# pscoro/JPEG-XL-Lossy-Image-Compression-Thesis

Measured on AMD Instinct MI355X. Metric: MPix/s VarDCT encode @ d1.0, 8K RGB, higher is better.
Workload: dtype f32; 1 GPU; 8k 7680x4320 RGB8 (synth_rgb8), VarDCT d1 e7, cjxl defaults (JXG_FLAGS_CJXL_DEFAULTS: Gaborish + EPF + masking AQ), proposals=0, ans-coded, 1 frame(s) per step, 2 distinct frames cycled, streaming entry points (jxg_submit_rgb8_device / jxg_receive, one host thread); global_batch=1, parallelism=frame-dp1

## Files before the change

jpeg-xl-lossy-image-compression-thesis_amd/csrc/jxg_encode.cpp:

```cpp
#include "jxg_ctx.h"

#include <cstdlib>
#include <cstring>

#include "jxg_codes.h"
#include "jxg_tables.h"

namespace jxg {

static void build_rows(const Frame& f, const Plan& P, std::vector<LfRow>& rows,
                       std::vector<LfChunk>& chunks, std::vector<uint32_t>& schunks) {
  rows.clear();
  chunks.clear();
  schunks.clear();
  auto add = [&](uint32_t lg, uint16_t stream, uint16_t ch, uint32_t y, uint32_t width) {
    for (uint32_t x0 = 0; x0 < width; x0 += kLfSeg) {
      const uint32_t wseg = std::min(kLfSeg, width - x0);
      const uint32_t sid = lg * 2 + stream;
      if (chunks.empty() || chunks.back().sid != sid || chunks.back().nrows == kLfChunkRows ||
          chunks.back().nsamp + wseg > kLfChunkSamples)
        chunks.push_back({(uint32_t)rows.size(), 0, sid, 0});
      chunks.back().nrows++;
      chunks.back().nsamp += wseg;
      rows.push_back({lg, stream, ch, y, x0, wseg, sid});
    }
  };
  for (uint32_t lg = 0; lg < f.nlf; lg++) {
    const uint32_t bx0 = (lg % f.lfxs) * 256, by0 = (lg / f.lfxs) * 256;
    const uint32_t bw = std::min(256u, f.bxs - bx0), bh = std::min(256u, f.bys - by0);
    const bool own = P.owns_lf(lg);
    schunks.push_back((uint32_t)chunks.size());
    if (own)
      for (uint16_t ch = 0; ch < 3; ch++)
        for (uint32_t y = 0; y < bh; y++) add(lg, 0, ch, y, bw);
    schunks.push_back((uint32_t)chunks.size());
    if (own) {
      const uint32_t cw = (bw + 7) / 8, chh = (bh + 7) / 8;
      for (uint16_t ch = 0; ch < 2; ch++)
        for (uint32_t y = 0; y < chh; y++) add(lg, 1, ch, y, cw);
      for (uint32_t y = 0; y < 2; y++) add(lg, 1, 2, y, bw * bh);
      for (uint32_t y = 0; y < bh; y++) add(lg, 1, 3, y, bw);
    }
  }
  schunks.push_back((uint32_t)chunks.size());
}

jxg_status wait_emission(Ctx* c, Job& J) {
  (void)J;
  JXG_HIP(hipStreamSynchronize(c->stream));
  return JXG_OK;
}

jxg_status stage_alloc(Ctx* c, Job& J) {
  hipStream_t s = c->stream;
  const jxg_params& P = c->params;
  const Frame& f = J.f;
  const size_t nb = (size_t)f.bxs * f.bys;
  J.homog = (P.proposals & 3u) != 0;
  J.ans = (P.flags & JXG_FLAG_ANS) != 0;
  J.lf = lf_code(P.flags, P.distance);
  jxg_status st = init_constants(c);
  if (st) return st;
  JXG_HIP(c->acs.ensure(nb));
  JXG_HIP(c->qf.ensure(nb));
  JXG_HIP(c->nz.ensure(nb * 3));
  JXG_HIP(c->dc.ensure(nb * 3));
  JXG_HIP(c->ac.ensure(nb * 192));
  if (J.homog) JXG_HIP(c->homog.ensure(nb * 3));
  J.max_s = P.effort >= 6 ? 8 : (P.effort >= 5 ? 4 : 0);
  const uint32_t ntiles = f.tiles_x * f.tiles_y;
  JXG_HIP(c->cmap.ensure((size_t)ntiles * 2));
  if (J.max_s) {
    JXG_HIP(c->ent.ensure(nb));
    JXG_HIP(c->xyb_tiles.ensure((size_t)ntiles * 3 * 4096));
    JXG_HIP(c->mcost.ensure((size_t)ntiles * kNumShapes * 32));
    JXG_HIP(c->mwork.ensure(1 + (size_t)ntiles * kNumShapes));
  }
  const bool new_plan = c->rows_w != J.w || c->rows_h != J.h || c->rows_rank != J.plan.rank ||
                        c->rows_world != J.plan.world;
  if (!J.plan.tiles.empty()) {
    JXG_HIP(c->tile_list.ensure(J.plan.tiles.size()));
    if (new_plan)
      JXG_HIP(hipMemcpyAsync(c->tile_list.p, J.plan.tiles.data(), J.plan.tiles.size() * 4,
                             hipMemcpyHostToDevice, s));
  }
  if (!J.plan.lf_mine.empty()) {
    JXG_HIP(c->lf_mine.ensure(J.plan.lf_mine.size()));
    if (new_plan)
      JXG_HIP(hipMemcpyAsync(c->lf_mine.p, J.plan.lf_mine.data(), J.plan.lf_mine.size(),
                             hipMemcpyHostToDevice, s));
  }
  JXG_HIP(c->vb.ensure((size_t)f.nlf * 65536));
  J.nstreams = f.nlf * 2;
  {
    const EncArenas::Layouts L = c->declare(f, J.plan.ng());
    JXG_HIP(c->stat.ensure(c->stat_bytes));
    JXG_HIP(c->h_stat.ensure(c->stat_bytes));
    JXG_HIP(c->up.ensure(c->up_bytes));
    JXG_HIP(c->h_up.ensure(c->up_bytes));
    JXG_HIP(c->bits.ensure(c->bits_bytes));
    JXG_HIP(c->h_bits.ensure(c->bits_bytes));
    L.stat.commit(c->stat.p, c->h_stat.p);
    L.up.commit(c->up.p, c->h_up.p);
    L.bits.commit(c->bits.p, c->h_bits.p);
  }
  if (new_plan) {
    build_rows(f, J.plan, c->rows_h_cache, c->chunks_h_cache, c->schunks_cache);
    c->rows_w = J.w;
    c->rows_h = J.h;
    c->rows_rank = J.plan.rank;
    c->rows_world = J.plan.world;
  }
  J.nrows = (uint32_t)c->rows_h_cache.size();
  J.nchunks = (uint32_t)c->chunks_h_cache.size();
  const uint32_t nstreams = J.nstreams;
  JXG_HIP(c->rows.ensure(J.nrows));
  JXG_HIP(c->lfchunks.ensure(J.nchunks));
  JXG_HIP(c->lfstatus.ensure(J.nchunks));
  JXG_HIP(c->stream_chunks.ensure(nstreams + 1));
  if (new_plan) {
    if (J.nrows)
      JXG_HIP(hipMemcpyAsync(c->rows.p, c->rows_h_cache.data(), J.nrows * sizeof(LfRow),
                             hipMemcpyHostToDevice, s));
    if (J.nchunks)
      JXG_HIP(hipMemcpyAsync(c->lfchunks.p, c->chunks_h_cache.data(), J.nchunks * sizeof(LfChunk),
                             hipMemcpyHostToDevice, s));
    JXG_HIP(hipMemcpyAsync(c->stream_chunks.p, c->schunks_cache.data(),
                           c->schunks_cache.size() * 4, hipMemcpyHostToDevice, s));
  }
// ... 748 lines not shown
```

jpeg-xl-lossy-image-compression-thesis_amd/csrc/jxg_kernels.h:

```cpp
#pragma once
#include <cmath>
#include <hip/hip_runtime.h>
#include <stddef.h>
#include <stdint.h>

#include "jxg_acmodel.h"
#include "jxg_decode_core.h"

namespace jxg {

constexpr uint32_t kMaxBatch = 4;
template <class A>
struct Batch {
  A a[kMaxBatch];
};
template <class A>
inline Batch<A> make_batch(const A* a, uint32_t k) {
  Batch<A> b{};
  for (uint32_t i = 0; i < k && i < kMaxBatch; i++) b.a[i] = a[i];
  return b;
}

struct FrontArgs {
  const uint8_t* rgb;
  uint32_t w, h;
  size_t stride;
  uint32_t bxs, bys, xp, yp, tiles_x;
  float distance;
  int effort;
  uint32_t proposals;
  int h1_int;
  int gab;
  float qf_base, inv_g;
  uint32_t G;
  float dc_mul[3], dc_step[3];
  uint8_t* acs;
  uint8_t* qf;
  int32_t* dc;
  int16_t* ac;
  uint16_t* nz;
  float* homog;
  float* ent;
  float* xyb_out;
  const uint32_t* tile_list;
  int8_t* cmap;
  uint32_t ntiles_all;
  uint4* zero;
  uint32_t zero_quads;
  const uint8_t* qf_in;
};
struct AqArgs {
  const uint8_t* rgb;
  uint32_t w, h;
  size_t stride;
  uint32_t xp, yp, bxs, bys, tiles_x;
  const float* lut;
  float ew[4];
  float mul, add, inv_g;
  uint8_t* qf;
  const uint32_t* tile_list;
};
void launch_aq(const AqArgs* a, uint32_t k, uint32_t ntiles, hipStream_t s);

constexpr int kNumKinds = 6;
constexpr int kKindOff[kNumKinds + 1] = {0, 128, 384, 896, 1920, 3968, 8064};
constexpr int kNumShapes = 9;
constexpr int kShapeOff[kNumShapes + 1] = {0, 128, 256, 512, 1024, 1536, 2560, 4608, 6656, 10752};
struct MergeArgs {
  const float* xyb;
  uint32_t bxs, bys, tiles_x, ntiles;
  const uint32_t* tile_list;
  uint32_t proposals;
  int max_s;
  uint32_t G;
  float dc_mul[3], dc_step[3];
  float* ent;
  const float* homog;
  uint8_t* acs;
  uint8_t* qf;
  int32_t* dc;
  int16_t* ac;
  uint16_t* nz;
  float* cost;
  const float* wk;
  const float* iwy;
  const float* sdk;
  const uint16_t* nat;
  uint32_t* work;
  uint32_t nwrite;
  const int8_t* cmap;
  uint32_t ntiles_all;
};
constexpr int kBigKindOff[5] = {0, 8192, 24576, 57344, 122880};
constexpr uint32_t kBigSlots = 512;
constexpr size_t kBigPlanes = 3 * 65536;
constexpr size_t kBigTabW = 0, kBigTabSd = 3 * 122880, kBigTabIw = 6 * 122880,
                 kBigTabLeeC = 7 * 122880, kBigTabLeeS = kBigTabLeeC + 9 * 128,
                 kBigTabLlfP = kBigTabLeeS + 9 * 256, kBigTabLlfIb = kBigTabLlfP + 6 * 32,
                 kBigTabFloats = kBigTabLlfIb + 6 * 32 * 32;
struct BigArgs {
  MergeArgs m;
  const float* tab;
  const uint16_t* nat;
  float* scratch;
  uint32_t slots;
  float* cost;
  uint32_t* work;
  uint32_t* kinds;
  const uint32_t* glist;
  uint32_t g0, ng, gxs;
};
hipError_t launch_big(const BigArgs* a, uint32_t k, hipStream_t s);

struct VbArgs {
  const uint8_t* acs;
  uint32_t bxs, bys, lfxs;
  const uint8_t* lf_mine;
  uint32_t* vb;
  uint32_t* count;
};
// ... 213 lines not shown
```

jpeg-xl-lossy-image-compression-thesis_amd/csrc/jxg_merge.hip:

```cpp
#include <float.h>

#include <cstdio>
#include <type_traits>

#include "jxg_device.h"
#include "jxg_kernels.h"
#include "jxg_lee_tables.h"

namespace jxg {

__constant__ float c_llf_p[4 * 8];
__constant__ float c_llf_ib[4 * 64];

constexpr int kMThreads = 256;
#ifndef JXG_MERGE_WPE
#define JXG_MERGE_WPE 4
#endif
#ifndef JXG_MERGE_WRITE_WPE
#define JXG_MERGE_WRITE_WPE 3
#endif
constexpr int kMS = 65;
constexpr int kMPlane = 64 * kMS;

template <int N>
// ... 47 lines not shown
    for (int k = 0; k < H - 1; k++) out(k, (t[k] + t[k + 1]) * kLeeS[l][2 * k + 1]);
    out(H - 1, t[H - 1] * kLeeS[l][N - 1]);
  }
}
template <class T>
__device__ __forceinline__ T dct64_first(T xi, T xm, int i, int h) {
  return dctN_first<64>(xi, xm, i, h);
}
template <class T, class Out>
__device__ __forceinline__ void dct64_rest(T* t, int h, Out out) {
  dctN_rest<64>(t, h, out);
}

#ifdef JXG_MERGE_PROFILE
__device__ unsigned long long g_mprof[16][8];
#define MPROF_MARK(k)                                                 \
  do {                                                                \
    if (!WRITE && threadIdx.x == 0) {                                 \
      const unsigned long long now_ = __builtin_readcyclecounter();   \
      if ((k) > 0) atomicAdd(&g_mprof[P.si][(k)], now_ - mprof_t0);   \
      mprof_t0 = now_;                                                \
    }                                                                 \
  } while (0)
#else
#define MPROF_MARK(k) \
  do {                \
  } while (0)
#endif

struct ShapeDesc {
  int type, lcy, lcx;
  float tmul;
};
constexpr ShapeDesc kShapes[kNumShapes] = {
    {6, 1, 0, 1.0f},   {7, 0, 1, 1.0f},   {4, 1, 1, 1.0f},
    {10, 2, 1, 1.02f}, {11, 1, 2, 1.02f}, {5, 2, 2, 1.03f},
    {19, 3, 2, 1.05f}, {20, 2, 3, 1.05f}, {18, 3, 3, 1.05f}};

__device__ __forceinline__ int bitlen_u(uint32_t v) { return 32 - __clz(v); }

struct MergeLds {
  float co[2 * kMPlane];
  float llf[3][64];
  float qsum[3][4][32];
  float btab[256];
  float vr3[32][3];
  int vbits[32];
  int vnz[32][3];
  int vraw[32];
  int valid[32];
  uint8_t braw[64];
  int any;
};
__device__ __forceinline__ float& llf_at(MergeLds& S, int c, int b) { return S.llf[c][b]; }
__device__ __forceinline__ int pass_src(int pass, int lc) { return pass ? 2 : 1 - lc; }
__device__ __forceinline__ int pass_plane(int pass, int lc) { return pass ? 1 : lc; }
__device__ __forceinline__ constexpr int chan_plane(int ch) { return ch == 1 ? 0 : 1; }

struct Pass {
  int si, type, lcy, lcx, soff, ls, tx, ty, tile;
  float tmul;
  __device__ __forceinline__ int cy() const { return 1 << lcy; }
  __device__ __forceinline__ int cx() const { return 1 << lcx; }
  __device__ __forceinline__ int R() const { return 8 << lcy; }
  __device__ __forceinline__ int C() const { return 8 << lcx; }
  __device__ __forceinline__ int lR() const { return 3 + lcy; }
  __device__ __forceinline__ int lC() const { return 3 + lcx; }
  __device__ __forceinline__ int lGX() const { return 3 - lcx; }
  __device__ __forceinline__ int lNV() const { return 6 - lcx - lcy; }
  __device__ __forceinline__ int NV() const { return 1 << lNV(); }
  __device__ __forceinline__ int bx0(int v) const { return (v & ((1 << lGX()) - 1)) << lcx; }
  __device__ __forceinline__ int by0(int v) const { return (v >> lGX()) << lcy; }
  __device__ __forceinline__ int off(int v, int plane) const {
    return plane * kMPlane + by0(v) * 8 * kMS + bx0(v) * 8;
  }
};

#ifndef JXG_MERGE_CHUNK
#define JXG_MERGE_CHUNK 32
#endif
__device__ __forceinline__ bool decode_wg(const MergeArgs& a, int& tile, int& si) {
  constexpr int T = JXG_MERGE_CHUNK;
  const int b = blockIdx.x, x = b & 7, q = b >> 3;
  const int r = q % (kNumShapes * T);
  si = r / T;
  tile = ((q / (kNumShapes * T)) * T + r % T) * 8 + x;
  if (tile >= (int)a.ntiles) return false;
  if (a.tile_list) tile = (int)a.tile_list[tile];
  return true;
}

__device__ __forceinline__ Pass make_pass(const MergeArgs& a, int tile, int si) {
  Pass P;
  P.si = si;
  const ShapeDesc& D = kShapes[si];
  P.type = D.type;
  P.lcy = D.lcy;
  P.lcx = D.lcx;
  P.tmul = D.tmul;
  P.soff = kShapeOff[si];
  P.ls = max(D.lcy, D.lcx);
  P.tile = tile;
  P.tx = tile % (int)a.tiles_x;
  P.ty = tile / (int)a.tiles_x;
  return P;
}

template <int C>
__device__ __forceinline__ void load_row(const float* src, float* d) {
#pragma unroll
  for (int q = 0; q < C / 4; q++) {
    const float4 u = reinterpret_cast<const float4*>(src)[q];
    d[4 * q] = u.x;
    d[4 * q + 1] = u.y;
    d[4 * q + 2] = u.z;
    d[4 * q + 3] = u.w;
  }
}
template <int C, int NCH>
__device__ __forceinline__ void row_pass(const MergeArgs& a, const Pass& P, MergeLds& S, int pass) {
  const float* tsrc = a.xyb + (size_t)P.tile * (3 * 4096);
  const int R = P.R(), lvr = P.lNV() + P.lR();
  if constexpr (C == 64) {
    const int npairs = NCH * P.NV() * R / 2;
    const int n = ((npairs + 63) >> 6) << 7;
    for (int i = threadIdx.x; i < n; i += kMThreads) {
      const int h = (i >> 6) & 1, pp = ((i >> 7) << 6) | (i & 63), r = pp * 2;
      if (pp >= npairs) continue;
      const int c = r >> lvr, v = (r >> P.lR()) & (P.NV() - 1), y = r & (R - 1);
      if (!S.valid[v]) continue;
      const float4* s0 =
          reinterpret_cast<const float4*>(tsrc + pass_src(pass, c) * 4096 + (P.by0(v) * 8 + y) * 64);
      const float4* s1 = s0 + 16;
      f2 t[32];
#pragma unroll
      for (int q = 0; q < 8; q++) {
        const float4 a0 = s0[q], b0 = s0[15 - q], a1 = s1[q], b1 = s1[15 - q];
        const float fa0[4] = {a0.x, a0.y, a0.z, a0.w}, fb0[4] = {b0.x, b0.y, b0.z, b0.w};
        const float fa1[4] = {a1.x, a1.y, a1.z, a1.w}, fb1[4] = {b1.x, b1.y, b1.z, b1.w};
#pragma unroll
        for (int j = 0; j < 4; j++)
          t[4 * q + j] = dct64_first(f2{fa0[j], fa1[j]}, f2{fb0[3 - j], fb1[3 - j]}, 4 * q + j, h);
      }
      const int off = P.off(v, pass_plane(pass, c)) + y * kMS;
      dct64_rest(t, h, [&](int k, f2 o) {
        S.co[off + 2 * k + h] = o.x;
        S.co[off + kMS + 2 * k + h] = o.y;
      });
    }
  } else {
    constexpr int PER = (NCH * 4096 / C + kMThreads - 1) / kMThreads;
    const int nrows = NCH * P.NV() * R;
    const int lgx = P.lGX();
    auto row_of = [&](int rr, int& c, int& v, int& y) {
      c = rr >> lvr;
      const int i = rr & ((1 << lvr) - 1);
      y = (i >> lgx) & (R - 1);
      v = ((i >> (lgx + P.lR())) << lgx) | (i & ((1 << lgx) - 1));
    };
    float buf[PER][C];
#pragma unroll
    for (int k = 0; k < PER; k++) {
      const int r = threadIdx.x + k * kMThreads;
      if (r < nrows) {
        int c, v, y;
        row_of(r, c, v, y);
        load_row<C>(tsrc + pass_src(pass, c) * 4096 + (P.by0(v) * 8 + y) * 64 + P.bx0(v) * 8,
                    buf[k]);
      } else {
#pragma unroll
        for (int q = 0; q < C; q++) buf[k][q] = 0.0f;
      }
    }
    constexpr int l = ilog2c<C>();
#pragma unroll
    for (int k = 0; k < PER; k += 2) {
      const int r0 = threadIdx.x + k * kMThreads, r1 = r0 + kMThreads;
      if (r0 >= nrows) continue;
      int c0, v0, y0, c1, v1, y1;
      row_of(r0, c0, v0, y0);
      row_of(r1, c1, v1, y1);
      const bool ok0 = S.valid[v0], ok1 = k + 1 < PER && r1 < nrows && S.valid[v1];
      if (!ok0 && !ok1) continue;
      if (k + 1 < PER) {
        f2 x[C];
#pragma unroll
        for (int q = 0; q < C; q++) x[q] = f2{buf[k][q], buf[k + 1][q]};
        lee<C>(x);
        const int off0 = P.off(v0, pass_plane(pass, c0)) + y0 * kMS,
                  off1 = P.off(v1, pass_plane(pass, c1)) + y1 * kMS;
#pragma unroll
        for (int q = 0; q < C; q++) {
          const f2 o = x[q] * kLeeS[l][q];
          if (ok0) S.co[off0 + q] = o.x;
          if (ok1) S.co[off1 + q] = o.y;
        }
      } else {
        float* x = buf[k];
        lee<C>(x);
        const int off0 = P.off(v0, pass_plane(pass, c0)) + y0 * kMS;
#pragma unroll
        for (int q = 0; q < C; q++) S.co[off0 + q] = x[q] * kLeeS[l][q];
      }
    }
  }
}

template <int R, int NCH>
__device__ __forceinline__ void col_pass(const Pass& P, MergeLds& S, int pass) {
  constexpr int lR = ilog2c<R>(), nb = 64 / R, lnb = 6 - lR;
  constexpr int npairs = NCH * nb * 32;
  const int lGX = P.lGX(), lC = P.lC();
  auto col_of = [&](int pidx, int& off, bool& okA, bool& okB) {
    const int X = pidx & 31, band = (pidx >> 5) & (nb - 1), c = pidx >> (5 + lnb);
    off = pass_plane(pass, c) * kMPlane + band * R * kMS + X;
    okA = S.valid[(band << lGX) | (X >> lC)];
    okB = S.valid[(band << lGX) | ((X + 32) >> lC)];
  };
  if constexpr (R == 64 || (R >= 16 && npairs <= kMThreads / 2)) {
    constexpr int H = R / 2;
    constexpr int n = ((npairs + 63) >> 6) << 7;
// ... 62 lines not shown
};
__device__ __forceinline__ int qtab_index(const Pass& P, int ky, int x) {
  return P.soff + ((ky >> 2) * P.C() + x) * 4;
}
template <int RPC, bool WRITE, int CH>
__device__ __forceinline__ void load_qtab(const MergeArgs& a, const Pass& P, QTab<RPC>& T) {
  constexpr int STOT = kShapeOff[kNumShapes];
#pragma unroll
  for (int it = 0; it < QTab<RPC>::NIT; it++) {
    const int j = threadIdx.x + it * kMThreads;
    const int ch = j >> (P.lNV() + P.lC()), x = j & (P.C() - 1);
#pragma unroll
    for (int kk = 0; kk < RPC; kk += 4) {
      const int ti = qtab_index(P, ch * RPC + kk, x);
      load_f<4>(a.wk + (size_t)CH * STOT + ti, &T.w[it][kk]);
      if (!WRITE) load_f<4>(a.sdk + (size_t)CH * STOT + ti, &T.sd[it][kk]);
      if (CH == 1) load_f<4>(a.iwy + ti, &T.iw[it][kk]);
    }
  }
}
template <int M>
__device__ __forceinline__ uint32_t grp_xor(uint32_t v) {
  if constexpr (M == 1) return (uint32_t)__builtin_amdgcn_mov_dpp((int)v, 0xB1, 0xF, 0xF, false);
  if constexpr (M == 2) return (uint32_t)__builtin_amdgcn_mov_dpp((int)v, 0x4E, 0xF, 0xF, false);
  if constexpr (M == 4) {
    const int t = __builtin_amdgcn_mov_dpp((int)v, 0x1B, 0xF, 0xF, false);
    return (uint32_t)__builtin_amdgcn_mov_dpp(t, 0x141, 0xF, 0xF, false);
  }
  if constexpr (M == 8) {
    const int t = __builtin_amdgcn_mov_dpp((int)v, 0x141, 0xF, 0xF, false);
    return (uint32_t)__builtin_amdgcn_mov_dpp(t, 0x140, 0xF, 0xF, false);
  }
  if constexpr (M == 16) return (uint32_t)__builtin_amdgcn_ds_swizzle((int)v, 0x401F);
  if constexpr (M == 32) {
    const uint32_t lo = (uint32_t)__builtin_amdgcn_readlane((int)v, 0);
    const uint32_t hi = (uint32_t)__builtin_amdgcn_readlane((int)v, 32);
    return (threadIdx.x & 32) ? lo : hi;
  }
}
template <int M>
__device__ __forceinline__ void grp_step(float& cp, int& packed) {
  cp += __uint_as_float(grp_xor<M>(__float_as_uint(cp)));
  packed += (int)grp_xor<M>((uint32_t)packed);
}
__device__ __forceinline__ void group_all_reduce(float& cp, int& packed, int C) {
  grp_step<1>(cp, packed);
  grp_step<2>(cp, packed);
  grp_step<4>(cp, packed);
  if (C > 8) grp_step<8>(cp, packed);
  if (C > 16) grp_step<16>(cp, packed);
  if (C > 32) grp_step<32>(cp, packed);
}

template <int RPC, bool WRITE, int CH>
__device__ __forceinline__ void quant_pass(const MergeArgs& a, const Pass& P, MergeLds& S, const QTab<RPC>& T) {
  constexpr int cidx = CH == 1 ? 0 : (CH == 0 ? 1 : 2);
  const int C = P.C(), NV = P.NV();
  float kc = 0.0f;
  if (CH != 1) {
    const float f = (float)a.cmap[(CH == 0 ? 0u : a.ntiles_all) + (uint32_t)P.tile];
    kc = CH == 0 ? f * (1.0f / 84.0f) : 1.0f + f * (1.0f / 84.0f);
  }
#pragma unroll
  for (int it = 0; it < QTab<RPC>::NIT; it++) {
    const int j = threadIdx.x + it * kMThreads;
    const int ch = j >> (P.lNV() + P.lC()), v = (j >> P.lC()) & (NV - 1), x = j & (C - 1);
    if (!S.valid[v]) continue;
    const int bx0 = P.bx0(v), by0 = P.by0(v);
    const float scale = (float)a.G * (float)S.vraw[v] / 65536.0f;
    float* cplane = S.co + P.off(v, chan_plane(CH)) + x;
    const float* yd = S.co + P.off(v, 0) + x;
    const float* w = T.w[it];
    const float* sd = T.sd[it];
    float iw[RPC];
    if (CH == 1) {
      const float inv_scale = 1.0f / scale;
#pragma unroll
      for (int kk = 0; kk < RPC; kk++) iw[kk] = T.iw[it][kk] * inv_scale;
    }
    uint16_t nat[RPC];
    if (WRITE) {
#pragma unroll
      for (int kk = 0; kk < RPC; kk += 4) {
        const uint2 u = *reinterpret_cast<const uint2*>(a.nat + qtab_index(P, ch * RPC + kk, x));
        nat[kk] = (uint16_t)u.x;
        nat[kk + 1] = (uint16_t)(u.x >> 16);
        nat[kk + 2] = (uint16_t)u.y;
        nat[kk + 3] = (uint16_t)(u.y >> 16);
      }
    }
    const bool llf_col = ch == 0 && x < P.cx();
    float cp = 0.0f;
    uint32_t eb8[2] = {0u, 0u};
#pragma unroll
    for (int kk = 0; kk < RPC; kk += 2) {
      const int ky = ch * RPC + kk;
      const f2 coef = f2{cplane[ky * kMS], cplane[(ky + 1) * kMS]};
      if (WRITE && llf_col) {
        if (kk < P.cy()) llf_at(S, CH, (by0 + ky) * 8 + bx0 + x) = coef.x;
        if (kk + 1 < P.cy()) llf_at(S, CH, (by0 + ky + 1) * 8 + bx0 + x) = coef.y;
      }
      f2 rv = coef;
      if (CH != 1) rv = rv - f2{kc, kc} * f2{yd[ky * kMS], yd[(ky + 1) * kMS]};
      const f2 vq = rv * (f2{w[kk], w[kk + 1]} * f2{scale, scale});
      float sqs[2], qfs[2];
#pragma unroll
      for (int h = 0; h < 2; h++) {
        const float vqh = h ? vq.y : vq.x;
        const float av = fabsf(vqh);
        qfs[h] = av < 0.58f ? 0.0f : floorf(fminf(av, 32767.0f) + 0.5f);
        sqs[h] = __builtin_copysignf(qfs[h], vqh);
      }
      if (CH == 1) {
        float adj[2];
#pragma unroll
        for (int h = 0; h < 2; h++) adj[h] = S.btab[min((int)qfs[h], 255)];
        if (__builtin_expect(__any(fmaxf(qfs[0], qfs[1]) >= 256.0f), 0)) {
#pragma unroll
          for (int h = 0; h < 2; h++)
            if (qfs[h] >= 256.0f) adj[h] = qfs[h] - 0.145f / qfs[h];
        }
#pragma unroll
        for (int h = 0; h < 2; h++) {
          const float a1 = __builtin_copysignf(adj[h], h ? vq.y : vq.x);
          cplane[(ky + h) * kMS] = a1 * iw[kk + h];
        }
      }
#pragma unroll
      for (int h = 0; h < 2; h++) {
        const float qf = qfs[h];
        eb8[kk >= 8] += __float_as_uint(qf) >> 23;
        if (WRITE) {
          const int qq = (int)sqs[h];
          const int p = nat[kk + h];
          const int sl = p >> 6;
          const int lbx = bx0 + (sl & (P.cx() - 1)), lby = by0 + (sl >> P.lcx);
          const size_t gb = (size_t)(P.ty * 8 + lby) * a.bxs + P.tx * 8 + lbx;
          a.ac[(gb * 3 + CH) * 64 + (p & 63)] = (int16_t)qq;
        }
      }
      if (!WRITE) {
        const f2 e = (vq - f2{sqs[0], sqs[1]}) * f2{sd[kk], sd[kk + 1]};
        cp = fmaf(e.x, e.x, cp);
        cp = fmaf(e.y, e.y, cp);
      }
    }
    const int nzc = (int)(eb8[0] / 127u) + (int)(eb8[1] / 127u);
    const int bits = 2 * (int)(eb8[0] + eb8[1]) - 250 * nzc;
    int packed = bits | nzc << 20;
    group_all_reduce(cp, packed, C);
    if (x == 0) {
      S.qsum[cidx][ch][v] = cp;
      if (packed & 0xFFFFF) atomicAdd(&S.vbits[v], packed & 0xFFFFF);
      if (packed >> 20) atomicAdd(&S.vnz[v][CH], packed >> 20);
    }
  }
}

template <bool WRITE>
__device__ __forceinline__ void transform_quant(const MergeArgs& a, const Pass& P, MergeLds& S) {
#ifdef JXG_MERGE_PROFILE
  unsigned long long mprof_t0 = 0;
#endif
  MPROF_MARK(0);
  auto transform = [&](auto nch_tag, int pass) {
    constexpr int NCH = decltype(nch_tag)::value;
    switch (P.lcx) {
      case 0: row_pass<8, NCH>(a, P, S, pass); break;
      case 1: row_pass<16, NCH>(a, P, S, pass); break;
      case 2: row_pass<32, NCH>(a, P, S, pass); break;
      default: row_pass<64, NCH>(a, P, S, pass); break;
    }
    __syncthreads();
    switch (P.lcy) {
      case 0: col_pass<8, NCH>(P, S, pass); break;
      case 1: col_pass<16, NCH>(P, S, pass); break;
      case 2: col_pass<32, NCH>(P, S, pass); break;
      default: col_pass<64, NCH>(P, S, pass); break;
    }
  };
  transform(std::integral_constant<int, 2>(), 0);
  MPROF_MARK(1);
  auto quant_yx = [&](auto rpc_tag) {
    constexpr int RPC = decltype(rpc_tag)::value;
    {
      QTab<RPC> ty;
      load_qtab<RPC, WRITE, 1>(a, P, ty);
      __syncthreads();
      MPROF_MARK(2);
      quant_pass<RPC, WRITE, 1>(a, P, S, ty);
    }
    QTab<RPC> tx;
    load_qtab<RPC, WRITE, 0>(a, P, tx);
    quant_pass<RPC, WRITE, 0>(a, P, S, tx);
  };
  auto quant_b = [&](auto rpc_tag) {
    constexpr int RPC = decltype(rpc_tag)::value;
    QTab<RPC> tb;
    load_qtab<RPC, WRITE, 2>(a, P, tb);
    __syncthreads();
    quant_pass<RPC, WRITE, 2>(a, P, S, tb);
  };
  if (P.lcy == 0) quant_yx(std::integral_constant<int, 8>());
  else quant_yx(std::integral_constant<int, 16>());
  __syncthreads();
  MPROF_MARK(3);
  transform(std::integral_constant<int, 1>(), 1);
  if (P.lcy == 0) quant_b(std::integral_constant<int, 8>());
  else quant_b(std::integral_constant<int, 16>());
  __syncthreads();
  MPROF_MARK(4);
}

__device__ __forceinline__ float varblock_dist(const Pass& P, const MergeLds& S, int v) {
  const int nch = P.lcy == 0 ? 1 : P.R() >> 4;
  float pc[3];
#pragma unroll
  for (int ci = 0; ci < 3; ci++) {
    float t = S.qsum[ci][0][v];
    for (int ch = 1; ch < nch; ch++) t = t + S.qsum[ci][ch][v];
    pc[ci] = t;
  }
  return (pc[0] + pc[1]) + pc[2];
}

template <bool WRITE>
__device__ __forceinline__ void setup_varblocks(const MergeArgs& a, const Pass& P, MergeLds& S,
                                                int nbx, int nby) {
  const int t = threadIdx.x;
  if (t < 64) {
    const int lbx = t & 7, lby = t >> 3;
    const bool in = lbx < nbx && lby < nby;
    const size_t gb = (size_t)(P.ty * 8 + lby) * a.bxs + P.tx * 8 + lbx;
    S.braw[t] = in ? a.qf[gb] : 0;
  }
  if (t < 32) {
    const int v = t;
    bool ok = false;
    if (v < P.NV()) {
      const int bx0 = P.bx0(v), by0 = P.by0(v);
      const size_t gb0 = (size_t)(P.ty * 8 + by0) * a.bxs + P.tx * 8 + bx0;
      if (WRITE) {
        ok = bx0 < nbx && by0 < nby && a.acs[gb0] == (uint8_t)P.type;
      } else {
        ok = (((bx0 >> P.ls) + 1) << P.ls) <= nbx && (((by0 >> P.ls) + 1) << P.ls) <= nby;
        if (ok && (a.proposals & 2u)) {
          S.vr3[v][0] = a.homog[gb0 * 3 + 0];
          S.vr3[v][1] = a.homog[gb0 * 3 + 1];
          S.vr3[v][2] = a.homog[gb0 * 3 + 2];
        }
      }
    }
    S.valid[v] = ok;
    S.vraw[v] = 0;
    S.vbits[v] = 0;
    S.vnz[v][0] = S.vnz[v][1] = S.vnz[v][2] = 0;
  }
  for (int i = t; i < 256; i += kMThreads)
    S.btab[i] = i == 0 ? 0.0f : (i == 1 ? 1.0f - 0.07005449891748593f : (float)i - 0.145f / (float)i);
}
__device__ __forceinline__ void vraw_pass(const MergeArgs& a, const Pass& P, MergeLds& S) {
  (void)a;
  const int b = threadIdx.x;
  if (b < 64) {
    const int lbx = b & 7, lby = b >> 3;
    const int v = ((lby >> P.lcy) << P.lGX()) | (lbx >> P.lcx);
    if (v < P.NV() && S.valid[v]) atomicMax(&S.vraw[v], (int)S.braw[b] + 1);
  }
}

__device__ __forceinline__ int max_level(const MergeArgs& a) {
  return a.max_s >= 8 ? 3 : (a.max_s >= 4 ? 2 : 1);
}

__global__ __launch_bounds__(kMThreads) __attribute__((amdgpu_waves_per_eu(JXG_MERGE_WPE)))
void merge_eval_kernel(Batch<MergeArgs> bt_) {
  const MergeArgs& a = bt_.a[blockIdx.z];
  __shared__ __attribute__((aligned(16))) MergeLds S;
  if (blockIdx.x == 0 && threadIdx.x == 0) a.work[0] = 0;
  int tile, si;
  if (!decode_wg(a, tile, si)) return;
  const Pass P = make_pass(a, tile, si);
  if (P.ls > max_level(a)) return;
  const int nbx = min(8, (int)a.bxs - P.tx * 8), nby = min(8, (int)a.bys - P.ty * 8);
  if ((1 << P.ls) > nbx || (1 << P.ls) > nby) return;
#ifdef JXG_MERGE_PROFILE
  const unsigned long long t_setup = __builtin_readcyclecounter();
#endif
  setup_varblocks<false>(a, P, S, nbx, nby);
  __syncthreads();
  vraw_pass(a, P, S);
#ifdef JXG_MERGE_PROFILE
  if (threadIdx.x == 0) atomicAdd(&g_mprof[P.si][5], __builtin_readcyclecounter() - t_setup);
#endif
  transform_quant<false>(a, P, S);
  const int v = threadIdx.x;
  if (v < P.NV() && S.valid[v]) {
    const float dist = varblock_dist(P, S, v);
    const int tb = bitlen_u((uint32_t)S.vnz[v][0]) + bitlen_u((uint32_t)S.vnz[v][1]) +
                   bitlen_u((uint32_t)S.vnz[v][2]);
    float e = ((float)(S.vbits[v] + tb) + 8.0f * dist) * P.tmul;
    if (a.proposals & 2u) e = hook_f(e, S.vr3[v][0], S.vr3[v][1], S.vr3[v][2]);
    a.cost[((size_t)tile * kNumShapes + si) * 32 + v] = e;
  }
}

constexpr int kResolveWaves = 16;
__device__ __forceinline__ void wave_sync_lds() {
  __builtin_amdgcn_fence(__ATOMIC_SEQ_CST, "wavefront");
  __builtin_amdgcn_wave_barrier();
}
__global__ __launch_bounds__(64 * kResolveWaves) void merge_resolve_kernel(Batch<MergeArgs> bt_) {
  const MergeArgs& a = bt_.a[blockIdx.z];
  __shared__ float sEntW[kResolveWaves][64];
  __shared__ uint8_t sAcsW[kResolveWaves][64];
  __shared__ uint32_t sCnt[kResolveWaves];
  __shared__ uint32_t sBase;
  const int wv = threadIdx.x >> 6, t = threadIdx.x & 63;
  float* sEnt = sEntW[wv];
  uint8_t* sAcs = sAcsW[wv];
  const int idx = blockIdx.x * kResolveWaves + wv;
  uint32_t has = 0;
  int tile = 0;
  if (idx < (int)a.ntiles) {
    tile = a.tile_list ? (int)a.tile_list[idx] : idx;
    const int tx = tile % (int)a.tiles_x, ty = tile / (int)a.tiles_x;
    const int nbx = min(8, (int)a.bxs - tx * 8), nby = min(8, (int)a.bys - ty * 8);
    const int lbx = t & 7, lby = t >> 3;
    const bool in = lbx < nbx && lby < nby;
    const size_t gb = (size_t)(ty * 8 + lby) * a.bxs + tx * 8 + lbx;
    sEnt[t] = in ? a.ent[gb] : 0.0f;
    sAcs[t] = in ? a.acs[gb] : 0;
    wave_sync_lds();
    const float* cost = a.cost + (size_t)tile * kNumShapes * 32;
    for (int s = 2; s <= a.max_s && s <= nbx && s <= nby; s *= 2) {
      const int nr = 8 / s;
      const int full = s == 2 ? 2 : (s == 4 ? 5 : 8);
      const int tall = s == 2 ? 0 : (s == 4 ? 3 : 6);
      if (t < nr * nr) {
        const int rx = t % nr, ry = t / nr;
        if ((rx + 1) * s <= nbx && (ry + 1) * s <= nby) {
          float cur = 0.0f;
          for (int iy = 0; iy < s; iy++)
            for (int ix = 0; ix < s; ix++) cur += sEnt[(ry * s + iy) * 8 + rx * s + ix];
          const int vf = ry * nr + rx, vl = ry * (16 / s) + 2 * rx, vt = (2 * ry) * nr + rx;
          const float e0 = cost[full * 32 + vf];
          const float el = cost[tall * 32 + vl], er = cost[tall * 32 + vl + 1];
          const float etop = cost[(tall + 1) * 32 + vt], ebot = cost[(tall + 1) * 32 + vt + nr];
          const float et = el + er, ew = etop + ebot;
          float best = cur;
          int choice = 0;
          if (!(e0 >= best)) {
            best = e0;
            choice = 1;
          }
          if (!(et >= best)) {
            best = et;
            choice = 2;
          }
          if (!(ew >= best)) {
            best = ew;
            choice = 3;
          }
          for (int j = 0; choice && j < (choice == 1 ? 1 : 2); j++) {
            int sh, bx, by;
            float e;
            if (choice == 1) {
              sh = full, bx = rx * s, by = ry * s, e = e0;
            } else if (choice == 2) {
              sh = tall, bx = rx * s + j * (s / 2), by = ry * s, e = j ? er : el;
            } else {
              sh = tall + 1, bx = rx * s, by = ry * s + j * (s / 2), e = j ? ebot : etop;
            }
            const int cy = 1 << kShapes[sh].lcy, cx = 1 << kShapes[sh].lcx;
            for (int iy = 0; iy < cy; iy++)
              for (int ix = 0; ix < cx; ix++) {
                const int b = (by + iy) * 8 + bx + ix;
                sAcs[b] = (uint8_t)(kShapes[sh].type | ((iy | ix) ? 0x80 : 0));
                sEnt[b] = (iy | ix) ? 0.0f : e;
              }
          }
        }
      }
      wave_sync_lds();
    }
    if (in) {
      a.acs[gb] = sAcs[t];
      a.ent[gb] = sEnt[t];
    }
    if (in && !(sAcs[t] & 0x80)) {
#pragma unroll
      for (int si = 0; si < kNumShapes; si++) has |= sAcs[t] == kShapes[si].type ? 1u << si : 0u;
    }
#pragma unroll
    for (int m = 1; m < 64; m <<= 1) has |= __shfl_xor(has, m, 64);
  }
  if (t == 0) sCnt[wv] = (uint32_t)__popc(has);
  __syncthreads();
  if (threadIdx.x == 0) {
    uint32_t tot = 0;
    for (int w = 0; w < kResolveWaves; w++) tot += sCnt[w];
    sBase = tot ? atomicAdd(a.work, tot) : 0u;
  }
  __syncthreads();
  uint32_t base = sBase;
  for (int w = 0; w < wv; w++) base += sCnt[w];
  if (t < kNumShapes && ((has >> t) & 1u))
    a.work[1 + base + __popc(has & ((1u << t) - 1u))] = (uint32_t)tile << 4 | (uint32_t)t;
}

__device__ __forceinline__ void write_entry(const MergeArgs& a, int tile, int si, MergeLds& S) {
  const Pass P = make_pass(a, tile, si);
  const int nbx = min(8, (int)a.bxs - P.tx * 8), nby = min(8, (int)a.bys - P.ty * 8);
  setup_varblocks<true>(a, P, S, nbx, nby);
  __syncthreads();
  vraw_pass(a, P, S);
  transform_quant<true>(a, P, S);
  const int cb = P.cy() * P.cx(), lcb = P.lcy + P.lcx;
  const size_t nb = (size_t)a.bxs * a.bys;
  const int ly = P.lcy, lx = P.lcx;
  for (int i = threadIdx.x; i < P.NV() * cb; i += kMThreads) {
    const int v = i >> lcb, k = i & (cb - 1);
    if (!S.valid[v]) continue;
    const int iy = k >> P.lcx, ix = k & (P.cx() - 1);
    const int bx0 = P.bx0(v), by0 = P.by0(v);
    const size_t gb = (size_t)(P.ty * 8 + by0 + iy) * a.bxs + P.tx * 8 + bx0 + ix;
    for (int c = 0; c < 3; c++) {
      const int n = S.vnz[v][c];
      a.nz[c * nb + gb] = (uint16_t)(k == 0 ? n : (n + cb - 1) >> lcb);
    }
    float px[8], py[8], ibx[8], iby[8];
#pragma unroll
    for (int k = 0; k < 8; k++) {
      px[k] = c_llf_p[lx * 8 + k];
      py[k] = c_llf_p[ly * 8 + k];
      ibx[k] = c_llf_ib[lx * 64 + ix * 8 + k];
      iby[k] = c_llf_ib[ly * 64 + iy * 8 + k];
    }
    const int cx = P.cx(), cy = P.cy();
    float dc[3];
#pragma unroll 1
    for (int c = 0; c < 3; c++) {
      float acc = 0.0f;
#pragma unroll
      for (int ky = 0; ky < 8; ky++) {
        if (ky < cy) {
          float u = 0.0f;
#pragma unroll
          for (int kx = 0; kx < 8; kx++) {
            if (kx < cx) {
              const float tt = (llf_at(S, c, (by0 + ky) * 8 + bx0 + kx) * py[ky]) * px[kx];
              u = fmaf(tt, ibx[kx], u);
            }
          }
          acc = fmaf(u, iby[ky], acc);
        }
      }
      dc[c] = acc;
    }
    int32_t q[3];
    quant_dc3(dc, a.dc_mul, a.dc_step, q);
    a.dc[gb] = q[0];
    a.dc[nb + gb] = q[1];
    a.dc[2 * nb + gb] = q[2];
    a.qf[gb] = (uint8_t)(S.vraw[v] - 1);
  }
}

__global__ __launch_bounds__(kMThreads) __attribute__((amdgpu_waves_per_eu(JXG_MERGE_WRITE_WPE)))
void merge_write_kernel(Batch<MergeArgs> bt_) {
  const MergeArgs& a = bt_.a[blockIdx.z];
  __shared__ __attribute__((aligned(16))) MergeLds S;
  const uint32_t n = __builtin_amdgcn_readfirstlane(*(volatile uint32_t*)a.work);
  for (uint32_t w = blockIdx.x; w < n; w += gridDim.x) {
    const uint32_t e = a.work[1 + w];
    write_entry(a, (int)(e >> 4), (int)(e & 15u), S);
    __syncthreads();
  }
}

__global__ __launch_bounds__(1024) void vb_list_kernel(Batch<VbArgs> bt_) {
  const VbArgs& a = bt_.a[blockIdx.z];
  __shared__ uint32_t sCnt[64 * 16];
  __shared__ uint32_t sWave[16];
  const uint32_t lg = blockIdx.x;
  if (a.lf_mine && !a.lf_mine[lg]) return;
  const uint32_t bx0 = (lg % a.lfxs) * 256, by0 = (lg / a.lfxs) * 256;
  const uint32_t bw = min(256u, a.bxs - bx0), bh = min(256u, a.bys - by0);
  const uint32_t n = bw * bh;
  const int lane = threadIdx.x & 63, wv = threadIdx.x >> 6;
  const uint64_t lt = (1ull << lane) - 1ull;
  const uint32_t dq = 1024u / bw, dr = 1024u % bw;
  const uint32_t y0 = threadIdx.x / bw, x0 = threadIdx.x % bw;
  auto step = [&](uint32_t& y, uint32_t& x) {
    x += dr;
    y += dq;
    if (x >= bw) {
      x -= bw;
      y++;
    }
  };
  uint64_t fl = 0;
  {
    uint32_t y = y0, x = x0;
#pragma unroll 16
    for (int k = 0; k < 64; k++) {
      const uint32_t i = (uint32_t)k * 1024 + threadIdx.x;
      if (i < n && !(a.acs[(size_t)(by0 + y) * a.bxs + bx0 + x] & 0x80)) fl |= 1ull << k;
      step(y, x);
    }
  }
  for (int k = 0; k < 64; k++) {
    const uint64_t bal = __ballot((fl >> k) & 1);
    if (lane == 0) sCnt[k * 16 + wv] = (uint32_t)__popcll(bal);
  }
  __syncthreads();
  const uint32_t v = sCnt[threadIdx.x];
  uint32_t incl = v;
#pragma unroll
  for (int d = 1; d < 64; d <<= 1) {
    const uint32_t t = __shfl_up(incl, d);
    if (lane >= d) incl += t;
  }
  if (lane == 63) sWave[wv] = incl;
  __syncthreads();
  uint32_t before = 0, total = 0;
  for (int w = 0; w < 16; w++) {
    before += w < wv ? sWave[w] : 0u;
    total += sWave[w];
// ... 58 lines not shown
```

Before: 10160 MPix/s.

## Pack same-shape varblocks from many tiles into dense merge-write work items

The merge resolve step now records each chosen varblock (tile plus block position) in a per-shape list with its own counter, replacing one (tile, shape) work entry per tile. The write kernel treats each slot as a varblock from any tile, filling up to the shape's slot count per pass, and carries per-slot source offsets, global block indices and colour-correlation factors in LDS. The aim is to avoid write passes where most of the varblock slots in a tile are invalid, so lanes stay busy and fewer passes run. It adds per-slot indirection, a nine-counter atomic layout, and a larger work buffer.

```diff
diff --git a/jpeg-xl-lossy-image-compression-thesis_amd/csrc/jxg_encode.cpp b/jpeg-xl-lossy-image-compression-thesis_amd/csrc/jxg_encode.cpp
--- a/jpeg-xl-lossy-image-compression-thesis_amd/csrc/jxg_encode.cpp
+++ b/jpeg-xl-lossy-image-compression-thesis_amd/csrc/jxg_encode.cpp
@@ -74,7 +74,7 @@
     JXG_HIP(c->ent.ensure(nb));
     JXG_HIP(c->xyb_tiles.ensure((size_t)ntiles * 3 * 4096));
     JXG_HIP(c->mcost.ensure((size_t)ntiles * kNumShapes * 32));
-    JXG_HIP(c->mwork.ensure(1 + (size_t)ntiles * kNumShapes));
+    JXG_HIP(c->mwork.ensure(merge_work_words(ntiles)));
   }
   const bool new_plan = c->rows_w != J.w || c->rows_h != J.h || c->rows_rank != J.plan.rank ||
                         c->rows_world != J.plan.world;
diff --git a/jpeg-xl-lossy-image-compression-thesis_amd/csrc/jxg_kernels.h b/jpeg-xl-lossy-image-compression-thesis_amd/csrc/jxg_kernels.h
--- a/jpeg-xl-lossy-image-compression-thesis_amd/csrc/jxg_kernels.h
+++ b/jpeg-xl-lossy-image-compression-thesis_amd/csrc/jxg_kernels.h
@@ -66,6 +66,13 @@
 constexpr int kKindOff[kNumKinds + 1] = {0, 128, 384, 896, 1920, 3968, 8064};
 constexpr int kNumShapes = 9;
 constexpr int kShapeOff[kNumShapes + 1] = {0, 128, 256, 512, 1024, 1536, 2560, 4608, 6656, 10752};
+constexpr int kMergeWorkHead = 16;
+constexpr int kShapeSlots[kNumShapes] = {32, 32, 16, 8, 8, 4, 2, 2, 1};
+constexpr int kShapeSlotOff[kNumShapes + 1] = {0, 32, 64, 80, 88, 96, 100, 102, 104, 105};
+constexpr size_t merge_list_off(int si, uint32_t ntiles) {
+  return kMergeWorkHead + (size_t)ntiles * kShapeSlotOff[si];
+}
+constexpr size_t merge_work_words(uint32_t ntiles) { return merge_list_off(kNumShapes, ntiles); }
 struct MergeArgs {
   const float* xyb;
   uint32_t bxs, bys, tiles_x, ntiles;
diff --git a/jpeg-xl-lossy-image-compression-thesis_amd/csrc/jxg_merge.hip b/jpeg-xl-lossy-image-compression-thesis_amd/csrc/jxg_merge.hip
--- a/jpeg-xl-lossy-image-compression-thesis_amd/csrc/jxg_merge.hip
+++ b/jpeg-xl-lossy-image-compression-thesis_amd/csrc/jxg_merge.hip
@@ -123,6 +123,13 @@
   uint8_t braw[64];
   int any;
 };
+struct WriteLds : MergeLds {
+  uint32_t ssrc[32];
+  uint32_t sgb[32];
+  float skc[2][32];
+};
+template <class L>
+constexpr bool kIsWrite = std::is_same<L, WriteLds>::value;
 __device__ __forceinline__ float& llf_at(MergeLds& S, int c, int b) { return S.llf[c][b]; }
 __device__ __forceinline__ int pass_src(int pass, int lc) { return pass ? 2 : 1 - lc; }
 __device__ __forceinline__ int pass_plane(int pass, int lc) { return pass ? 1 : lc; }
@@ -188,8 +195,9 @@
     d[4 * q + 3] = u.w;
   }
 }
-template <int C, int NCH>
-__device__ __forceinline__ void row_pass(const MergeArgs& a, const Pass& P, MergeLds& S, int pass) {
+template <int C, int NCH, class L>
+__device__ __forceinline__ void row_pass(const MergeArgs& a, const Pass& P, L& S, int pass) {
+  constexpr bool WRITE = kIsWrite<L>;
   const float* tsrc = a.xyb + (size_t)P.tile * (3 * 4096);
   const int R = P.R(), lvr = P.lNV() + P.lR();
   if constexpr (C == 64) {
@@ -200,8 +208,10 @@
       if (pp >= npairs) continue;
       const int c = r >> lvr, v = (r >> P.lR()) & (P.NV() - 1), y = r & (R - 1);
       if (!S.valid[v]) continue;
-      const float4* s0 =
-          reinterpret_cast<const float4*>(tsrc + pass_src(pass, c) * 4096 + (P.by0(v) * 8 + y) * 64);
+      const float* src0;
+      if constexpr (WRITE) src0 = a.xyb + S.ssrc[v] + pass_src(pass, c) * 4096 + y * 64;
+      else src0 = tsrc + pass_src(pass, c) * 4096 + (P.by0(v) * 8 + y) * 64;
+      const float4* s0 = reinterpret_cast<const float4*>(src0);
       const float4* s1 = s0 + 16;
       f2 t[32];
 #pragma unroll
@@ -236,8 +246,11 @@
       if (r < nrows) {
         int c, v, y;
         row_of(r, c, v, y);
-        load_row<C>(tsrc + pass_src(pass, c) * 4096 + (P.by0(v) * 8 + y) * 64 + P.bx0(v) * 8,
-                    buf[k]);
+        if constexpr (WRITE)
+          load_row<C>(a.xyb + S.ssrc[v] + pass_src(pass, c) * 4096 + y * 64, buf[k]);
+        else
+          load_row<C>(tsrc + pass_src(pass, c) * 4096 + (P.by0(v) * 8 + y) * 64 + P.bx0(v) * 8,
+                      buf[k]);
       } else {
 #pragma unroll
         for (int q = 0; q < C; q++) buf[k][q] = 0.0f;
@@ -406,12 +419,13 @@
   if (C > 32) grp_step<32>(cp, packed);
 }
 
-template <int RPC, bool WRITE, int CH>
-__device__ __forceinline__ void quant_pass(const MergeArgs& a, const Pass& P, MergeLds& S, const QTab<RPC>& T) {
+template <int RPC, bool WRITE, int CH, class L>
+__device__ __forceinline__ void quant_pass(const MergeArgs& a, const Pass& P, L& S, const QTab<RPC>& T) {
+  static_assert(WRITE == kIsWrite<L>, "the write kernel's LDS carries the per-slot arrays");
   constexpr int cidx = CH == 1 ? 0 : (CH == 0 ? 1 : 2);
   const int C = P.C(), NV = P.NV();
   float kc = 0.0f;
-  if (CH != 1) {
+  if (!WRITE && CH != 1) {
     const float f = (float)a.cmap[(CH == 0 ? 0u : a.ntiles_all) + (uint32_t)P.tile];
     kc = CH == 0 ? f * (1.0f / 84.0f) : 1.0f + f * (1.0f / 84.0f);
   }
@@ -421,6 +435,7 @@
     const int ch = j >> (P.lNV() + P.lC()), v = (j >> P.lC()) & (NV - 1), x = j & (C - 1);
     if (!S.valid[v]) continue;
     const int bx0 = P.bx0(v), by0 = P.by0(v);
+    if constexpr (WRITE && CH != 1) kc = S.skc[CH == 0 ? 0 : 1][v];
     const float scale = (float)a.G * (float)S.vraw[v] / 65536.0f;
     float* cplane = S.co + P.off(v, chan_plane(CH)) + x;
     const float* yd = S.co + P.off(v, 0) + x;
@@ -488,9 +503,10 @@
           const int qq = (int)sqs[h];
           const int p = nat[kk + h];
           const int sl = p >> 6;
-          const int lbx = bx0 + (sl & (P.cx() - 1)), lby = by0 + (sl >> P.lcx);
-          const size_t gb = (size_t)(P.ty * 8 + lby) * a.bxs + P.tx * 8 + lbx;
-          a.ac[(gb * 3 + CH) * 64 + (p & 63)] = (int16_t)qq;
+          if constexpr (WRITE) {
+            const size_t gb = (size_t)S.sgb[v] + (size_t)(sl >> P.lcx) * a.bxs + (sl & (P.cx() - 1));
+            a.ac[(gb * 3 + CH) * 64 + (p & 63)] = (int16_t)qq;
+          }
         }
       }
       if (!WRITE) {
@@ -511,8 +527,8 @@
   }
 }
 
-template <bool WRITE>
-__device__ __forceinline__ void transform_quant(const MergeArgs& a, const Pass& P, MergeLds& S) {
+template <bool WRITE, class L>
+__device__ __forceinline__ void transform_quant(const MergeArgs& a, const Pass& P, L& S) {
 #ifdef JXG_MERGE_PROFILE
   unsigned long long mprof_t0 = 0;
 #endif
@@ -578,7 +594,10 @@
   return (pc[0] + pc[1]) + pc[2];
 }
 
-template <bool WRITE>
+__device__ __forceinline__ void fill_btab(MergeLds& S) {
+  for (int i = threadIdx.x; i < 256; i += kMThreads)
+    S.btab[i] = i == 0 ? 0.0f : (i == 1 ? 1.0f - 0.07005449891748593f : (float)i - 0.145f / (float)i);
+}
 __device__ __forceinline__ void setup_varblocks(const MergeArgs& a, const Pass& P, MergeLds& S,
                                                 int nbx, int nby) {
   const int t = threadIdx.x;
@@ -594,15 +613,11 @@
     if (v < P.NV()) {
       const int bx0 = P.bx0(v), by0 = P.by0(v);
       const size_t gb0 = (size_t)(P.ty * 8 + by0) * a.bxs + P.tx * 8 + bx0;
-      if (WRITE) {
-        ok = bx0 < nbx && by0 < nby && a.acs[gb0] == (uint8_t)P.type;
-      } else {
-        ok = (((bx0 >> P.ls) + 1) << P.ls) <= nbx && (((by0 >> P.ls) + 1) << P.ls) <= nby;
-        if (ok && (a.proposals & 2u)) {
-          S.vr3[v][0] = a.homog[gb0 * 3 + 0];
-          S.vr3[v][1] = a.homog[gb0 * 3 + 1];
-          S.vr3[v][2] = a.homog[gb0 * 3 + 2];
-        }
+      ok = (((bx0 >> P.ls) + 1) << P.ls) <= nbx && (((by0 >> P.ls) + 1) << P.ls) <= nby;
+      if (ok && (a.proposals & 2u)) {
+        S.vr3[v][0] = a.homog[gb0 * 3 + 0];
+        S.vr3[v][1] = a.homog[gb0 * 3 + 1];
+        S.vr3[v][2] = a.homog[gb0 * 3 + 2];
       }
     }
     S.valid[v] = ok;
@@ -610,8 +625,7 @@
     S.vbits[v] = 0;
     S.vnz[v][0] = S.vnz[v][1] = S.vnz[v][2] = 0;
   }
-  for (int i = t; i < 256; i += kMThreads)
-    S.btab[i] = i == 0 ? 0.0f : (i == 1 ? 1.0f - 0.07005449891748593f : (float)i - 0.145f / (float)i);
+  fill_btab(S);
 }
 __device__ __forceinline__ void vraw_pass(const MergeArgs& a, const Pass& P, MergeLds& S) {
   (void)a;
@@ -622,6 +636,44 @@
     if (v < P.NV() && S.valid[v]) atomicMax(&S.vraw[v], (int)S.braw[b] + 1);
   }
 }
+__device__ __forceinline__ void setup_slots(const MergeArgs& a, const Pass& P, WriteLds& S,
+                                            const uint32_t* list, uint32_t first, uint32_t n) {
+  (void)P;
+  const int v = threadIdx.x;
+  if (v < 32) {
+    const bool ok = (uint32_t)v < n;
+    uint32_t src = 0, gb0 = 0;
+    float kx = 0.0f, kb = 0.0f;
+    if (ok) {
+      const uint32_t e = list[first + v], tile = e >> 6, by = (e >> 3) & 7u, bx = e & 7u;
+      const uint32_t tx = tile % a.tiles_x, ty = tile / a.tiles_x;
+      src = tile * (3u * 4096u) + by * (8u * 64u) + bx * 8u;
+      gb0 = (ty * 8u + by) * a.bxs + tx * 8u + bx;
+      kx = (float)a.cmap[tile] * (1.0f / 84.0f);
+      kb = 1.0f + (float)a.cmap[a.ntiles_all + tile] * (1.0f / 84.0f);
+    }
+    S.ssrc[v] = src;
+    S.sgb[v] = gb0;
+    S.skc[0][v] = kx;
+    S.skc[1][v] = kb;
+    S.valid[v] = ok;
+    S.vraw[v] = 0;
+    S.vbits[v] = 0;
+    S.vnz[v][0] = S.vnz[v][1] = S.vnz[v][2] = 0;
+  }
+  fill_btab(S);
+}
+__device__ __forceinline__ void vraw_slots(const MergeArgs& a, const Pass& P, WriteLds& S) {
+  const int b = threadIdx.x;
+  if (b < 64) {
+    const int lbx = b & 7, lby = b >> 3;
+    const int v = ((lby >> P.lcy) << P.lGX()) | (lbx >> P.lcx);
+    if (v < P.NV() && S.valid[v]) {
+      const size_t gb = (size_t)S.sgb[v] + (size_t)(lby & (P.cy() - 1)) * a.bxs + (lbx & (P.cx() - 1));
+      atomicMax(&S.vraw[v], (int)a.qf[gb] + 1);
+    }
+  }
+}
 
 __device__ __forceinline__ int max_level(const MergeArgs& a) {
   return a.max_s >= 8 ? 3 : (a.max_s >= 4 ? 2 : 1);
@@ -631,7 +683,7 @@
 void merge_eval_kernel(Batch<MergeArgs> bt_) {
   const MergeArgs& a = bt_.a[blockIdx.z];
   __shared__ __attribute__((aligned(16))) MergeLds S;
-  if (blockIdx.x == 0 && threadIdx.x == 0) a.work[0] = 0;
+  if (blockIdx.x == 0 && threadIdx.x < kNumShapes) a.work[threadIdx.x] = 0;
   int tile, si;
   if (!decode_wg(a, tile, si)) return;
   const Pass P = make_pass(a, tile, si);
@@ -641,7 +693,7 @@
 #ifdef JXG_MERGE_PROFILE
   const unsigned long long t_setup = __builtin_readcyclecounter();
 #endif
-  setup_varblocks<false>(a, P, S, nbx, nby);
+  setup_varblocks(a, P, S, nbx, nby);
   __syncthreads();
   vraw_pass(a, P, S);
 #ifdef JXG_MERGE_PROFILE
@@ -668,13 +720,12 @@
   const MergeArgs& a = bt_.a[blockIdx.z];
   __shared__ float sEntW[kResolveWaves][64];
   __shared__ uint8_t sAcsW[kResolveWaves][64];
-  __shared__ uint32_t sCnt[kResolveWaves];
-  __shared__ uint32_t sBase;
+  __shared__ uint32_t sCnt[kResolveWaves][kNumShapes];
   const int wv = threadIdx.x >> 6, t = threadIdx.x & 63;
   float* sEnt = sEntW[wv];
   uint8_t* sAcs = sAcsW[wv];
   const int idx = blockIdx.x * kResolveWaves + wv;
-  uint32_t has = 0;
+  int my = -1;
   int tile = 0;
   if (idx < (int)a.ntiles) {
     tile = a.tile_list ? (int)a.tile_list[idx] : idx;
@@ -744,31 +795,39 @@
     }
     if (in && !(sAcs[t] & 0x80)) {
 #pragma unroll
-      for (int si = 0; si < kNumShapes; si++) has |= sAcs[t] == kShapes[si].type ? 1u << si : 0u;
-    }
-#pragma unroll
-    for (int m = 1; m < 64; m <<= 1) has |= __shfl_xor(has, m, 64);
-  }
-  if (t == 0) sCnt[wv] = (uint32_t)__popc(has);
+      for (int si = 0; si < kNumShapes; si++) my = sAcs[t] == kShapes[si].type ? si : my;
+    }
+  }
+  uint32_t rank = 0;
+#pragma unroll
+  for (int si = 0; si < kNumShapes; si++) {
+    const uint64_t bal = __ballot(my == si);
+    if (t == 0) sCnt[wv][si] = (uint32_t)__popcll(bal);
+    if (my == si) rank = (uint32_t)__popcll(bal & ((1ull << t) - 1ull));
+  }
   __syncthreads();
-  if (threadIdx.x == 0) {
+  if (threadIdx.x < kNumShapes) {
+    const int si = threadIdx.x;
     uint32_t tot = 0;
-    for (int w = 0; w < kResolveWaves; w++) tot += sCnt[w];
-    sBase = tot ? atomicAdd(a.work, tot) : 0u;
+    for (int w = 0; w < kResolveWaves; w++) tot += sCnt[w][si];
+    uint32_t base = tot ? atomicAdd(a.work + si, tot) : 0u;
+    for (int w = 0; w < kResolveWaves; w++) {
+      const uint32_t n = sCnt[w][si];
+      sCnt[w][si] = base;
+      base += n;
+    }
   }
   __syncthreads();
-  uint32_t base = sBase;
-  for (int w = 0; w < wv; w++) base += sCnt[w];
-  if (t < kNumShapes && ((has >> t) & 1u))
-    a.work[1 + base + __popc(has & ((1u << t) - 1u))] = (uint32_t)tile << 4 | (uint32_t)t;
-}
-
-__device__ __forceinline__ void write_entry(const MergeArgs& a, int tile, int si, MergeLds& S) {
-  const Pass P = make_pass(a, tile, si);
-  const int nbx = min(8, (int)a.bxs - P.tx * 8), nby = min(8, (int)a.bys - P.ty * 8);
-  setup_varblocks<true>(a, P, S, nbx, nby);
+  if (my >= 0)
+    a.work[merge_list_off(my, a.ntiles) + sCnt[wv][my] + rank] = (uint32_t)tile << 6 | (uint32_t)t;
+}
+
+__device__ __forceinline__ void write_pass(const MergeArgs& a, int si, uint32_t first, uint32_t n,
+                                           WriteLds& S) {
+  const Pass P = make_pass(a, 0, si);
+  setup_slots(a, P, S, a.work + merge_list_off(si, a.ntiles), first, n);
   __syncthreads();
-  vraw_pass(a, P, S);
+  vraw_slots(a, P, S);
   transform_quant<true>(a, P, S);
   const int cb = P.cy() * P.cx(), lcb = P.lcy + P.lcx;
   const size_t nb = (size_t)a.bxs * a.bys;
@@ -778,7 +837,7 @@
     if (!S.valid[v]) continue;
     const int iy = k >> P.lcx, ix = k & (P.cx() - 1);
     const int bx0 = P.bx0(v), by0 = P.by0(v);
-    const size_t gb = (size_t)(P.ty * 8 + by0 + iy) * a.bxs + P.tx * 8 + bx0 + ix;
+    const size_t gb = (size_t)S.sgb[v] + (size_t)iy * a.bxs + ix;
     for (int c = 0; c < 3; c++) {
       const int n = S.vnz[v][c];
       a.nz[c * nb + gb] = (uint16_t)(k == 0 ? n : (n + cb - 1) >> lcb);
@@ -824,11 +883,27 @@
 __global__ __launch_bounds__(kMThreads) __attribute__((amdgpu_waves_per_eu(JXG_MERGE_WRITE_WPE)))
 void merge_write_kernel(Batch<MergeArgs> bt_) {
   const MergeArgs& a = bt_.a[blockIdx.z];
-  __shared__ __attribute__((aligned(16))) MergeLds S;
-  const uint32_t n = __builtin_amdgcn_readfirstlane(*(volatile uint32_t*)a.work);
-  for (uint32_t w = blockIdx.x; w < n; w += gridDim.x) {
-    const uint32_t e = a.work[1 + w];
-    write_entry(a, (int)(e >> 4), (int)(e & 15u), S);
+  __shared__ __attribute__((aligned(16))) WriteLds S;
+  uint32_t cnt[kNumShapes], total = 0;
+#pragma unroll
+  for (int si = 0; si < kNumShapes; si++) {
+    cnt[si] = __builtin_amdgcn_readfirstlane(((volatile uint32_t*)a.work)[si]);
+    total += (cnt[si] + kShapeSlots[si] - 1) / kShapeSlots[si];
+  }
+  for (uint32_t w = blockIdx.x; w < total; w += gridDim.x) {
+    int si = 0;
+    uint32_t first = 0, n = 0, start = 0;
+#pragma unroll
+    for (int j = kNumShapes - 1; j >= 0; j--) {
+      const uint32_t np = (cnt[j] + kShapeSlots[j] - 1) / kShapeSlots[j];
+      if (w >= start && w - start < np) {
+        si = j;
+        first = (w - start) * kShapeSlots[j];
+        n = min((uint32_t)kShapeSlots[j], cnt[j] - first);
+      }
+      start += np;
+    }
+    write_pass(a, si, first, n, S);
     __syncthreads();
   }
 }
```

Measured after the change: 10580 MPix/s, median of 6. +4.1%, better.
